# ETH3D/badslam

Measured on AMD Instinct MI355X. Metric: BA iterations/sec (and ms/iter) at N keyframes x M surfels, 640x480, higher is better.
Workload: dtype f32

## Files before the change

badslam_amd/capi.py:

```python
import ctypes as C
import os

_HERE = os.path.dirname(os.path.abspath(__file__))
LIB_PATH = os.path.join(os.environ.get("BADSLAM_LIB_DIR") or os.path.join(_HERE, "lib"), "libbadslam_hip.so")

SURFEL_ATTRIBUTE_COUNT = 17
MERGE_BUFFER_COUNT = 3
KF_ACTIVE, KF_COVISIBLE_ACTIVE, KF_INACTIVE = 0, 1, 2
ARITHMETIC_EXACT, ARITHMETIC_FAST = 0, 1

SURFEL_X, SURFEL_Y, SURFEL_Z, SURFEL_NORMAL, SURFEL_RADIUS_SQUARED, SURFEL_COLOR, SURFEL_DESCRIPTOR1, SURFEL_DESCRIPTOR2 = range(8)
SURFEL_ACCUM0 = 8


class BackendError(RuntimeError):
    pass


class Camera(C.Structure):
    _fields_ = [("fx", C.c_float), ("fy", C.c_float), ("cx", C.c_float), ("cy", C.c_float),
                ("width", C.c_int32), ("height", C.c_int32)]


class DepthParams(C.Structure):
# ... 186 lines not shown
                                             C.POINTER(C.c_uint32), C.POINTER(C.c_uint32)]),
    "bahip_extract_surfel_shard": (C.c_int, [C.c_void_p, C.POINTER(Surfels), C.c_int, C.c_int, C.c_uint32, C.POINTER(Surfels), C.POINTER(C.c_uint32)]),
    "bahip_debug_set_intrinsics_bin_capacity": (C.c_int, [C.c_void_p, C.c_int]),
    "bahip_debug_intrinsics_bin_stats": (C.c_int, [C.c_void_p, C.POINTER(C.c_uint32), C.POINTER(C.c_uint32), C.POINTER(C.c_uint64)]),
    "bahip_debug_set_intrinsics_slices": (C.c_int, [C.c_void_p, C.c_int]),
    "bahip_debug_read_intrinsics_sums": (C.c_int, [C.c_void_p, C.POINTER(C.c_float), C.POINTER(C.c_float)]),
    "bahip_exchange_stats": (C.c_int, [C.c_void_p, C.POINTER(C.c_longlong), C.POINTER(C.c_longlong), C.c_int]),
    "bahip_context_set_lifecycle_dealing": (C.c_int, [C.c_void_p, C.c_int]),
    "bahip_debug_lifecycle_deal_stats": (C.c_int, [C.c_void_p, C.POINTER(C.c_longlong), C.c_int]),
    "bahip_debug_exact_sum": (C.c_int, [C.c_void_p, C.POINTER(C.c_float), C.c_size_t, C.c_int, C.POINTER(C.c_double)]),
    "bahip_debug_count_pairs": (C.c_int, [C.c_void_p, C.POINTER(Surfels), C.POINTER(C.c_uint64)]),
    "bahip_debug_set_launch_shapes": (C.c_int, [C.c_int, C.c_int]),
    "bahip_debug_set_pose_form": (C.c_int, [C.c_int]),
    "bahip_debug_set_append_groups": (C.c_int, [C.c_int]),
    "bahip_debug_geometry_hybrid_launches": (C.c_int, [C.POINTER(C.c_longlong)]),
    "bahip_debug_set_creation_chain": (C.c_int, [C.c_int]),
    "bahip_debug_creation_chain_batches": (C.c_int, [C.POINTER(C.c_longlong)]),
    "bahip_debug_set_merge_cells": (C.c_int, [C.c_int]),
    "bahip_debug_merge_cells_batches": (C.c_int, [C.POINTER(C.c_longlong)]),
    "bahip_debug_set_pose_lds_items": (C.c_int, [C.c_int]),
    "bahip_debug_set_pose_lds_shape": (C.c_int, [C.c_int, C.c_int]),
    "bahip_debug_set_fused_iteration_begin": (C.c_int, [C.c_int]),
    "bahip_debug_set_intrinsics_reduce_form": (C.c_int, [C.c_int]),
    "bahip_debug_set_pose_rounds_ahead": (C.c_int, [C.c_int]),
    "bahip_debug_set_device_loop": (C.c_int, [C.c_int]),
    "bahip_debug_alternating_loop_calls": (C.c_int, [C.POINTER(C.c_longlong), C.POINTER(C.c_longlong)]),
    "bahip_debug_set_pcg_lds_form": (C.c_int, [C.c_int]),
    "bahip_debug_pose_form_launches": (C.c_int, [C.POINTER(C.c_longlong), C.POINTER(C.c_longlong), C.c_int]),
    "bahip_debug_pose_kernel_dispatches": (C.c_int, [C.POINTER(C.c_longlong)]),
    "bahip_debug_live_allocations": (C.c_int, [C.POINTER(C.c_longlong), C.POINTER(C.c_longlong)]),
# ... 40 lines not shown
```

badslam_amd/csrc/ba_launch.h:

```cpp
#pragma once

#include "ba_device.h"
#include <cstdlib>

inline int bahip_env_int(const char* name, int fallback) {
  const char* e = std::getenv(name);
  return e ? std::atoi(e) : fallback;
}

#ifdef BAHIP_FAST_MATH
#define BAHIP_FLAVOUR fast
#else
#define BAHIP_FLAVOUR exact
#endif
#define BAHIP_FLAVOURED_BEGIN namespace bahip { namespace BAHIP_FLAVOUR {
#define BAHIP_FLAVOURED_END } }

namespace bahip {

struct SupportingView {
  uint32_t* b[BAHIP_MERGE_BUFFER_COUNT];
  uint32_t pitch;
};

// ... 65 lines not shown
                       int update_activation, int round, void* host_out,
                       int sequence ,
                       const PoseLoopControl* loop = nullptr);
void launch_pose_init_from_keyframes(hipStream_t stream, const KfEntry* frames, int num_kfs, void* work, HbFixed* Hb, void* host_out,
                                     int kf_rank = 0, int kf_world = 1 ,
                                     const int* stop = nullptr);

void launch_window_activation(hipStream_t stream, KfEntry* frames, int num_kfs, const uint8_t* in_window, const int* offsets,
                              const int* indices, const int* stop = nullptr);
void launch_propagate_covisible(hipStream_t stream, KfEntry* frames, int num_kfs, const int* offsets, const int* indices,
                                const int* stop = nullptr);
bool launch_iteration_begin(hipStream_t stream, KfEntry* frames, int num_kfs, int mode, const uint8_t* in_window, const int* offsets, const int* indices,
                            void* work, HbFixed* Hb, void* host_out, const int* stop);

void set_tile_waves(int waves);
long long geometry_hybrid_launches();
void set_pose_lds_waves(int waves);
void set_pose_lds_parts_shift(int shift);
void set_pose_lds_items(int items);
void pcg_step1_form_launches(long long out[2]);
long long pose_kernel_dispatches();
void pose_form_launches(long long out[2], bool reset);
void set_pose_form(int form);
void set_pose_parts(int parts);
void launch_jacobian_debug(hipStream_t stream, int kind, const float* in, float* out);
void launch_pose_step_debug(hipStream_t stream, const float* in, float* out);
void launch_exact_math_debug(hipStream_t stream, int kind, const float* in, float* out, size_t n);
void launch_pose_limbs_debug(hipStream_t stream, const float* in, long long* out, size_t n);
void launch_wave_reduce_debug(hipStream_t stream, const float* in, float* out);
void launch_evaluate_pairs(hipStream_t stream, const Intrinsics& in, const KfEntry& frame, const SurfelsView& s,
// ... 170 lines not shown


#define BAHIP_FLAVOURED_DECLARATIONS                                                                                                          \
                                                                                                                      \
  void launch_activation(hipStream_t stream, const Intrinsics& in, const KfEntry* kfs, int num_kfs, const SurfelsView& s, uint32_t surfels_size); \
  void launch_normals(hipStream_t stream, const Intrinsics& in, const KfEntry* kfs, int num_kfs, const SurfelsView& s);                       \
  void launch_geometry(hipStream_t stream, bool use_depth, bool use_desc, const Intrinsics& in, const KfEntry* kfs, int num_kfs,              \
                       const SurfelsView& s, long long activate_count, const uint32_t* sched, const int* stop);                              \
  void launch_geometry_phase(hipStream_t stream, int phase, bool use_depth, bool use_desc, const Intrinsics& in, const KfEntry* kfs,          \
                             int num_kfs, const SurfelsView& s, long long activate_count, const ClassPartials& cpn, const ClassPartials& cpp); \
  void launch_activation_hits(hipStream_t stream, const Intrinsics& in, const KfEntry* kfs, int num_kfs, const SurfelsView& s,                \
                              uint32_t surfels_size, int kf_rank, int kf_world, uint32_t* hits);                                              \
  void launch_normals_phase(hipStream_t stream, int phase, const Intrinsics& in, const KfEntry* kfs, int num_kfs, const SurfelsView& s,      \
                            const ClassPartials& cp);                                                                                         \
  void set_tile_waves(int waves);                                                                                                             \
  long long geometry_hybrid_launches();                                                                                                       \
                                                                                                                        \
  void launch_pose_accumulate(hipStream_t stream, bool use_depth, bool use_desc, const Intrinsics& in, const KfEntry* frames,                 \
                              const void* work, int num_work, const SurfelsView& s, HbFixed* Hb, void* tile_bounds, bool stored_bounds,       \
                              int num_listed, uint32_t* tile_counters, int* parity_inout, uint32_t* tile_cost, const uint32_t* sched,         \
                              const int* listed_count, const int* stop);                                                                      \
  bool pose_round_can_be_queued_ahead(uint32_t surfels, int num_items, bool have_tile_counters);                                              \
  void set_pose_lds_waves(int waves);                                                                                                         \
  void set_pose_lds_parts_shift(int shift);                                                                                                   \
  void set_pose_lds_items(int items);                                                                                                         \
  long long pose_kernel_dispatches();                                                                                                         \
  void pose_form_launches(long long out[2], bool reset);                                                                                      \
  void set_pose_form(int form);                                                                                                               \
  void set_pose_parts(int parts);                                                                                                             \
  void launch_evaluate_pairs(hipStream_t stream, const Intrinsics& in, const KfEntry& frame, const SurfelsView& s, const uint32_t* indices,   \
// ... 77 lines not shown
```

badslam_amd/csrc/capi.hip:

```cpp
#include "capi_internal.h"

using namespace bahip;
using namespace bahip_capi;

namespace bahip_capi {

thread_local std::string g_last_error;

int fail(const char* what, const char* file, int line, hipError_t e) {
  char buf[512];
  if (e != hipSuccess) snprintf(buf, sizeof(buf), "%s failed at %s:%d: %s", what, file, line, hipGetErrorString(e));
  else snprintf(buf, sizeof(buf), "%s (%s:%d)", what, file, line);
  g_last_error = buf;
  return 1;
}

Intrinsics make_intrinsics(const bahip_camera& cc, const bahip_camera& dc, const bahip_depth_params& dp) {
  Intrinsics in{};
  in.fx = dc.fx; in.fy = dc.fy; in.cx = dc.cx; in.cy = dc.cy;
  in.fx_inv = 1.0f / dc.fx;
  in.fy_inv = 1.0f / dc.fy;
  const float cx_pixel_center = dc.cx - 0.5f, cy_pixel_center = dc.cy - 0.5f;
  in.cx_inv = -cx_pixel_center * in.fx_inv;
  in.cy_inv = -cy_pixel_center * in.fy_inv;
// ... 195 lines not shown
  if (!ctx) return;
  hipStreamSynchronize(ctx->stream);
#ifdef BAHIP_COUNT_CANDIDATES
  bahip::pose_counters_dump();
#endif
#ifdef BAHIP_TILE_TIMELINE
  if (const char* dir = getenv("BAHIP_TIMELINE_DIR")) {
    bahip::geometry_timeline_dump((std::string(dir) + "/geometry_timeline.bin").c_str());
    bahip::pose_timeline_dump((std::string(dir) + "/pose_timeline.bin").c_str());
  }
#endif
  if (ctx->intr_aux_stream) { hipStreamDestroy(ctx->intr_aux_stream); for (hipEvent_t e : ctx->intr_events) if (e) hipEventDestroy(e); }
  stage_free(&ctx->stage_kfs); stage_free(&ctx->stage_covis); stage_free(&ctx->stage_window); stage_free(&ctx->stage_gather);
  rccl_destroy_communicator(ctx);
  for (auto& t : ctx->timers) for (auto e : t.ev) hipEventDestroy(e);
  delete ctx;
}

int bahip_context_synchronize(bahip_context* ctx) {
  HIP_TRY(hipStreamSynchronize(ctx->stream));
  return 0;
}

int bahip_context_take_capacity_exceeded(bahip_context* ctx) {
  const int flag = ctx->capacity_exceeded ? 1 : 0;
  ctx->capacity_exceeded = false;
  return flag;
}

int bahip_malloc_pitch(void** ptr, size_t* pitch_bytes, size_t width_bytes, size_t height) {
// ... 292 lines not shown
```

badslam_amd/csrc/capi_debug.hip:

```cpp
#include "capi_internal.h"

using namespace bahip;
using namespace bahip_capi;

static const char* const kHookScratch = "the scratch of a test hook";

extern "C" {
int bahip_debug_live_allocations(long long* count_out, long long* bytes_out) {
  if (count_out) *count_out = g_live_allocations.load();
  if (bytes_out) *bytes_out = g_live_bytes.load();
  return 0;
}

int bahip_debug_evaluate_pairs(bahip_context* ctx, const bahip_frame* frame, const float frame_T_global[12],
                               const bahip_surfels* surfels, const uint32_t* surfel_indices_host, int count, float* out_host) {
  REQUIRE(ctx->have_intrinsics, "bahip_set_intrinsics not called");
  if (count <= 0) return 0;
  KfEntry e;
  if (make_entry(ctx, *frame, 0, &e)) return 1;
  memcpy(e.pose.F, frame_T_global, 12 * sizeof(float));
  DeviceBuffer<uint32_t> idx; DeviceBuffer<float> out;
  if (idx.reserve(count, 0, kHookScratch) || out.reserve(40 * (size_t)count, 0, kHookScratch)) return 1;
  HIP_TRY(hipMemcpy(idx, surfel_indices_host, sizeof(uint32_t) * count, hipMemcpyHostToDevice));
  launch_evaluate_pairs(ctx->stream, ctx->in, e, make_view(surfels), idx, count, out);
// ... 94 lines not shown
  REQUIRE(form == 0 || form == 1 || form == 2, "pose form must be 0 (automatic), 1 (one tile per wavefront, global atomics) or 2 (persistent, LDS table)");
  set_pose_form(form);
  return 0;
}

int bahip_debug_set_launch_shapes(int tile_waves, int pose_parts) {
  REQUIRE(tile_waves == 0 || tile_waves == 1 || tile_waves == 4 || tile_waves == 5, "tile_waves must be 0 (automatic), 1, 4 or 5 (the geometry step's hybrid shape)");
  REQUIRE(pose_parts == 0 || pose_parts == 1 || pose_parts == 2 || pose_parts == 4 || pose_parts == 8, "pose_parts must be 0, 1, 2, 4 or 8");
  set_tile_waves(tile_waves);
  set_pose_parts(pose_parts);
  return 0;
}

int bahip_debug_geometry_hybrid_launches(long long* launches_out) { if (launches_out) *launches_out = geometry_hybrid_launches(); return 0; }

int bahip_debug_jacobian(bahip_context* ctx, int kind, const float* in, int n_in, float* out, int n_out) {
  REQUIRE(kind >= 0 && kind <= 4 && n_in > 0 && n_in <= 16 && n_out > 0 && n_out <= 8, "bahip_debug_jacobian: bad arguments");
  DeviceBuffer<float> d_in, d_out;
  if (d_in.reserve(16, 0, kHookScratch) || d_out.reserve(8, 0, kHookScratch)) return 1;
  HIP_TRY(hipMemcpyAsync(d_in, in, n_in * sizeof(float), hipMemcpyHostToDevice, ctx->stream));
  launch_jacobian_debug(ctx->stream, kind, d_in, d_out);
  CHECK_LAUNCH();
  HIP_TRY(hipMemcpyAsync(out, d_out, n_out * sizeof(float), hipMemcpyDeviceToHost, ctx->stream));
  HIP_TRY(hipStreamSynchronize(ctx->stream));
  return 0;
}

int bahip_debug_read_pattern(bahip_context* ctx, size_t bytes, int pattern, int repeats) {
  REQUIRE(bytes >= 4096 && (pattern == 0 || pattern == 1) && repeats >= 1, "bahip_debug_read_pattern: bad arguments");
  DeviceBuffer<void> buf;
// ... 123 lines not shown
```

badslam_amd/csrc/capi_internal.h:

```cpp
#pragma once

#include <dlfcn.h>
#include <stdio.h>
#include <stdlib.h>
#include <string.h>

#include <atomic>
#include <chrono>
#include <memory>
#include <thread>

#include <string>
#include <vector>

#include "ba_launch.h"
#include "capi_buffers.h"
#include "exact_sum.h"
#include "ldlt.h"
#include "se3_device.h"

namespace bahip_capi {
using namespace bahip;

int fail(const char* what, const char* file, int line, hipError_t e = hipSuccess);
// ... 87 lines not shown
  DeviceBuffer<uint32_t> merge_planes[BAHIP_MERGE_BUFFER_COUNT];
  const void* supporting_planes_empty = nullptr;
  bool row_major_creation = false;
  bool poll_disabled = false;
  DeviceBuffer<void> dev_lifecycle_bounds;
  size_t lifecycle_bounds_capacity = 0;
  uint32_t lifecycle_bounds_tiles = 0;
  const void* lifecycle_bounds_data = nullptr;
  std::vector<float> lifecycle_frames;
  std::vector<uint32_t> lifecycle_list_offsets, lifecycle_list_counts;
  DeviceBuffer<float> dev_lifecycle_frames;
  DeviceBuffer<uint32_t> dev_lifecycle_cursors;
  DeviceBuffer<uint32_t> dev_lifecycle_lists;
  DeviceBuffer<void> dev_tile_bounds;
  DeviceBuffer<uint32_t> dev_tile_cost, dev_tile_order;
  size_t tile_schedule_capacity = 0;
  uint32_t tile_order_tiles = 0;
  int phases_since_schedule = 0;
  uint32_t tile_order_unavailable_tiles = 0;
  bool tile_order_unavailable_for(uint32_t padded_tiles) const { return padded_tiles != 0 && tile_order_unavailable_tiles == padded_tiles; }
  DeviceBuffer<int> dev_loop_ctl;
  PinnedBuffer<int> host_loop_ctl{kHostVisible};
  int rounds_hint_table = 1, rounds_hint_frame = 1;

  DeviceBuffer<void> intr_scratch;
  int intr_capacity = 0;
  DeviceBuffer<uint32_t> intr_bin_cursors;
  DeviceBuffer<uint32_t> intr_bin_records;
  PinnedBuffer<uint32_t> intr_bin_counts_host;
  int intr_bin_count = 0;
// ... 100 lines not shown
```

badslam_amd/csrc/kernels_surfel.hip:

```cpp
#include <stdlib.h>
#include <cstdio>

#include "ba_device.h"
#include "ba_launch.h"
#include "wave_cull.h"

namespace bahip {

#ifndef BAHIP_WAVES_ATTR
#define BAHIP_WAVES_ATTR __attribute__((amdgpu_waves_per_eu(4)))
#endif
constexpr int kSurfelBlock = 64;
constexpr int kMaxSumClasses = 8;

enum SumsMode { kSumsFused = 0, kSumsProduce = 1, kSumsConsume = 2 };
__device__ __forceinline__ bool position_valid(Vec3 p) { return p.x == p.x; }
static inline unsigned grid_for(uint32_t n) { return xcd_padded_tiles((n + kSurfelBlock - 1) / kSurfelBlock); }
#if defined(BAHIP_TILE_TIMELINE) && !defined(BAHIP_FAST_MATH)
__device__ unsigned long long g_geometry_timeline[65536][2];
void geometry_timeline_dump(const char* path) {
  static unsigned long long host[65536][2];
  if (hipMemcpyFromSymbol(host, HIP_SYMBOL(g_geometry_timeline), sizeof(host)) != hipSuccess) return;
  if (FILE* f = fopen(path, "wb")) { fwrite(host, sizeof(host), 1, f); fclose(f); }
}
// ... 75 lines not shown
  bool active = false;
  for_each_candidate_until(
      num_kfs,
      [&](int k) { return kfs[k].activation == BAHIP_KF_ACTIVE && sphere_may_project(in, kfs[k].pose.F, wb); },
      [&](int k) {
        if (in_range && !active) {
          Assoc r;
          if (project_associate<false>(in, kfs[k].pose.F, kfs[k].geom, gp, gn, &r, nullptr)) active = true;
        }
        return __all(active || !in_range) != 0;
      });
  if (in_range) s.active[i] = (s.active[i] & (uint8_t)~kSurfelActiveFlag) | (active ? kSurfelActiveFlag : 0);
}

constexpr int kMaskChunks = 4;
template <int kWaves, bool kActivate, int kMode = kSumsFused>
__device__ __forceinline__ void normals_pass(const Intrinsics& in, const KfEntry* __restrict__ kfs, int num_kfs,
                                             const WaveBounds& wb, SurfelsView& s, uint32_t i, bool* live_inout, bool decide,
                                             Vec3 gp, Vec3* gn_inout, float* lds, const ClassPartials& cp = ClassPartials{},
                                             bool in_range = false, unsigned long long* masks = nullptr) {
  const bool writer = kWaves == 1 || (threadIdx.x >> 6) == 0;
  const Vec3 gn = *gn_inout;
  bool live = *live_inout;
  constexpr int kCount = kActivate ? 5 : 4;
  float sum[kCount];
  tile_sums<kWaves, kCount, kMode>(sum, lds, [&](float (&acc)[kCount], int cls) {
    struct Started { Projected p; PixelWords pix; };
    for_each_candidate_pipelined<Started>(
        num_kfs,
        [&](int k) {
          float f[12];
          int32_t activation;
          load_candidate(kfs[k].pose.F, &kfs[k].activation, f, &activation);
          return activation != BAHIP_KF_INACTIVE && sphere_may_project(in, f, wb);
        },
        [&](int k) {
          Started st;
          st.p = project_surfel(in, kfs[k].pose.F, gp);
          st.pix = load_pixel_words(in, kfs[k].geom, st.p);
          return st;
        },
        [&](int k, const Started& st) {
          const Projected& p = st.p;
          const PixelWords& pix = st.pix;
          Assoc r;
          const bool associated = live && associate_from_words<false>(in, kfs[k].pose.F, gn, p, pix, &r, nullptr);
          gathers_arrived(pix);
          if (associated) {
            const Vec3 g = mul33(kfs[k].pose.GR, unpack_normal8(r.normal_bits));
            acc[0] += g.x; acc[1] += g.y; acc[2] += g.z; acc[3] += 1.f;
            if (kActivate) acc[kCount - 1] += (kfs[k].activation == BAHIP_KF_ACTIVE) ? 1.f : 0.f;
          }
        },
        in.sum_classes, cls, masks ? masks + cls * kMaskChunks : nullptr, masks ? kMaskChunks : 0, false);
  }, in.sum_classes, cp, i, in_range);
  if (kMode == kSumsProduce) return;
  if (kActivate && decide) {
    const bool active = live && sum[kCount - 1] >= 1.f;
    if (writer) s.active[i] = (s.active[i] & (uint8_t)~kSurfelActiveFlag) | (active ? kSurfelActiveFlag : 0);
    live = active;
    *live_inout = active;
  }
  if (!live) return;
  const float sx = sum[0], sy = sum[1], sz = sum[2], count = sum[3];
  if (count >= 1) {
    const uint32_t packed = pack_normal10((1.f / count) * mk3(sx, sy, sz));
    if (writer) reinterpret_cast<uint32_t*>(s.row(kSurfelNormal))[i] = packed;
    *gn_inout = unpack_normal10(packed);
  }
}

template <int kWaves>
__global__ void __launch_bounds__(64 * kWaves) BAHIP_WAVES_ATTR
normals_kernel(Intrinsics in, const KfEntry* __restrict__ kfs, int num_kfs, SurfelsView s) {
  __shared__ float lds[kWaves == 1 ? 1 : kMaxSumClasses * 4 * 64];
  const int lane = threadIdx.x & 63;
  const uint32_t i = xcd_chunked_tile(blockIdx.x) * kSurfelBlock + lane;
  const bool in_range = i < s.size;
  const uint32_t ii = in_range ? i : 0;
  bool live = in_range && (s.active[ii] & kSurfelActiveFlag);
  const Vec3 gp = surfel_position(s, ii);
  Vec3 gn = surfel_normal(s, ii);
  const WaveBounds wb = wave_bounds(gp, live && position_valid(gp));
  normals_pass<kWaves, false>(in, kfs, num_kfs, wb, s, ii, &live, false, gp, &gn, lds);
}

template <bool kUseDepth, bool kUseDesc, int kWaves, bool kActivate, int kPhase>
__device__ __forceinline__ void geometry_step(const Intrinsics& in, const KfEntry* __restrict__ kfs, int num_kfs, SurfelsView& s,
                                              uint32_t activate_count, float* lds, const ClassPartials& cpn, const ClassPartials& cpp,
                                              uint32_t tile , unsigned long long* replay_masks) {
  constexpr int kNormalsMode = kPhase == 1 ? kSumsProduce : kPhase == 2 ? kSumsConsume : kSumsFused;
  constexpr int kPositionMode = kPhase == 2 ? kSumsProduce : kPhase == 3 ? kSumsConsume : kSumsFused;
  const int lane = threadIdx.x & 63;
  const bool writer = kWaves == 1 || (threadIdx.x >> 6) == 0;
  const uint32_t i = tile * kSurfelBlock + lane;
  const bool in_range = i < s.size;
  const uint32_t ii = in_range ? i : 0;
  const bool decide = kActivate && kPhase != 3 && in_range && i < activate_count;
  bool live = in_range && (decide || (s.active[ii] & kSurfelActiveFlag));
  const Vec3 gp = surfel_position(s, ii);
  Vec3 gn = surfel_normal(s, ii);
  const WaveBounds wb = wave_bounds(gp, live && position_valid(gp));
  if (wb.r < 0.f) {
    if (decide && writer && kPhase != 1) s.active[ii] = s.active[ii] & (uint8_t)~kSurfelActiveFlag;
    return;
  }
  constexpr bool kReplayMasks = kWaves == 1 && kPhase == 0;
  unsigned long long* masks = kReplayMasks ? replay_masks : nullptr;
  if (kPhase != 3) normals_pass<kWaves, kActivate, kNormalsMode>(in, kfs, num_kfs, wb, s, ii, &live, decide, gp, &gn, lds, cpn, in_range, masks);
  if (kPhase == 1) return;

  auto cand = [&](int k) {
    float f[12];
    int32_t activation;
    load_candidate(kfs[k].pose.F, &kfs[k].activation, f, &activation);
    return activation != BAHIP_KF_INACTIVE && sphere_may_project(in, f, wb);
  };

  if (!kUseDesc) {
    float hb[2];
    tile_sums<kWaves, 2, kPositionMode>(hb, lds, [&](float (&acc)[2], int cls) {
      for_each_candidate_cached(num_kfs, cand, [&](int k) {
        const Projected p = project_surfel(in, kfs[k].pose.F, gp);
        const PixelWords pix = load_pixel_words(in, kfs[k].geom, p);
// ... 98 lines not shown
  const float x2 = y2 / H22;
  const float x1 = (y1 - H12 * x2) / H11;
  const float x0 = (y0 - H02 * x2 - H01 * x1) / H00;
  if (x0 != 0) {
    const Vec3 np = gp - x0 * gn;
    s.row(kSurfelX)[i] = np.x; s.row(kSurfelY)[i] = np.y; s.row(kSurfelZ)[i] = np.z;
  }
  if (x1 != 0) s.row(kSurfelDescriptor1)[i] = fmaxf(-180.f, fminf(180.f, d1 - x1));
  if (x2 != 0) s.row(kSurfelDescriptor2)[i] = fmaxf(-180.f, fminf(180.f, d2 - x2));
}


template <bool kUseDepth, bool kUseDesc, int kWaves, bool kActivate>
__global__ void __launch_bounds__(64 * kWaves) BAHIP_WAVES_ATTR
geometry_kernel(Intrinsics in, const KfEntry* __restrict__ kfs, int num_kfs, SurfelsView s, uint32_t activate_count,
                const uint32_t* __restrict__ sched, const int* __restrict__ stop ) {
  __shared__ float lds[kWaves == 1 ? 1 : kMaxSumClasses * 8 * 64];
  __shared__ unsigned long long candidate_masks[kWaves == 1 ? kMaxSumClasses * kMaskChunks : 1];
  if (stop && load_global(stop) != 0) return;
#ifdef BAHIP_RECORD_GEOMETRY_TIMELINE
  const unsigned long long t0 = wall_clock64();
#endif
  uint32_t tile;
  if (!scheduled_tile(blockIdx.x, gridDim.x - (sched ? kHeavySlots : 0u), sched, &tile)) return;
  geometry_step<kUseDepth, kUseDesc, kWaves, kActivate, 0>(in, kfs, num_kfs, s, activate_count, lds, ClassPartials{}, ClassPartials{}, tile, candidate_masks);
#ifdef BAHIP_RECORD_GEOMETRY_TIMELINE
  if (threadIdx.x == 0 && blockIdx.x < 65536) { g_geometry_timeline[blockIdx.x][0] = t0; g_geometry_timeline[blockIdx.x][1] = wall_clock64(); }
#endif
}

#ifndef BAHIP_HYBRID_WAVES
#define BAHIP_HYBRID_WAVES 4
#endif
template <bool kUseDepth, bool kUseDesc, bool kActivate>
__global__ void __launch_bounds__(256) __attribute__((amdgpu_waves_per_eu(BAHIP_HYBRID_WAVES)))
geometry_hybrid_kernel(Intrinsics in, const KfEntry* __restrict__ kfs, int num_kfs, SurfelsView s, uint32_t activate_count,
                       const uint32_t* __restrict__ sched , uint32_t padded_tiles, const int* __restrict__ stop) {
  __shared__ float lds[kMaxSumClasses * 8 * 64];
  __shared__ unsigned long long candidate_masks[4][kMaxSumClasses * kMaskChunks];
  if (stop && load_global(stop) != 0) return;
// ... 51 lines not shown
          if (project_associate<false>(in, kfs[k].pose.F, kfs[k].geom, gp, gn, &r, nullptr)) active = true;
        }
        return __all(active || !in_range) != 0;
      });
  if (in_range) hits[i] = active ? 1u : 0u;
}
void launch_activation(hipStream_t stream, const Intrinsics& in, const KfEntry* kfs, int num_kfs, const SurfelsView& s,
                       uint32_t surfels_size) {
  if (surfels_size == 0) return;
  hipLaunchKernelGGL(activation_kernel, dim3(grid_for(surfels_size)), dim3(kSurfelBlock), 0, stream, in, kfs, num_kfs, s,
                     surfels_size);
}

static int g_forced_tile_waves = bahip_env_int("BAHIP_TILE_WAVES", 0);
static long long g_geometry_hybrid_launches = 0;
long long geometry_hybrid_launches() { return g_geometry_hybrid_launches; }
void set_tile_waves(int waves) { g_forced_tile_waves = waves; }
static int tile_waves(uint32_t surfels) {
  const int forced = g_forced_tile_waves;
  if (forced == 1 || forced == 4) return forced;
  return grid_for(surfels) >= 8192 ? 1 : 4;
}

void launch_normals(hipStream_t stream, const Intrinsics& in, const KfEntry* kfs, int num_kfs, const SurfelsView& s) {
  if (s.size == 0) return;
  const dim3 grid(grid_for(s.size));
  switch (tile_waves(s.size)) {
    case 1: hipLaunchKernelGGL(normals_kernel<1>, grid, dim3(64), 0, stream, in, kfs, num_kfs, s); break;
    default: hipLaunchKernelGGL(normals_kernel<4>, grid, dim3(256), 0, stream, in, kfs, num_kfs, s); break;
  }
}

template <int kWaves, bool kActivate>
static void launch_geometry_shape(hipStream_t stream, bool use_depth, bool use_desc, const Intrinsics& in, const KfEntry* kfs,
                                  int num_kfs, const SurfelsView& s, uint32_t activate_count, const uint32_t* sched, const int* stop) {
  const dim3 grid(sched_positions(grid_for(s.size), sched)), block(64 * kWaves);
  if (!use_desc) hipLaunchKernelGGL((geometry_kernel<true, false, kWaves, kActivate>), grid, block, 0, stream, in, kfs, num_kfs, s, activate_count, sched, stop);
  else if (use_depth) hipLaunchKernelGGL((geometry_kernel<true, true, kWaves, kActivate>), grid, block, 0, stream, in, kfs, num_kfs, s, activate_count, sched, stop);
  else hipLaunchKernelGGL((geometry_kernel<false, true, kWaves, kActivate>), grid, block, 0, stream, in, kfs, num_kfs, s, activate_count, sched, stop);
}

template <bool kActivate>
static void launch_geometry_hybrid(hipStream_t stream, bool use_depth, bool use_desc, const Intrinsics& in, const KfEntry* kfs,
                                   int num_kfs, const SurfelsView& s, uint32_t activate_count, const uint32_t* sched, const int* stop) {
  const uint32_t padded = grid_for(s.size);
  const dim3 grid(kHeavySlots + (padded + 3u) / 4u), block(256);
  if (!use_desc) hipLaunchKernelGGL((geometry_hybrid_kernel<true, false, kActivate>), grid, block, 0, stream, in, kfs, num_kfs, s, activate_count, sched, padded, stop);
  else if (use_depth) hipLaunchKernelGGL((geometry_hybrid_kernel<true, true, kActivate>), grid, block, 0, stream, in, kfs, num_kfs, s, activate_count, sched, padded, stop);
  else hipLaunchKernelGGL((geometry_hybrid_kernel<false, true, kActivate>), grid, block, 0, stream, in, kfs, num_kfs, s, activate_count, sched, padded, stop);
}

void launch_geometry(hipStream_t stream, bool use_depth, bool use_desc, const Intrinsics& in, const KfEntry* kfs,
                     int num_kfs, const SurfelsView& s, long long activate_count, const uint32_t* sched, const int* stop) {
  if (s.size == 0) return;
// ... 141 lines not shown
                     long long activate_count, const uint32_t* sched, const int* stop) {
  BAHIP_PICK(in, launch_geometry(stream, use_depth, use_desc, in, kfs, num_kfs, s, activate_count, sched, stop));
}
void launch_geometry_phase(hipStream_t stream, int phase, bool use_depth, bool use_desc, const Intrinsics& in, const KfEntry* kfs, int num_kfs,
                           const SurfelsView& s, long long activate_count, const ClassPartials& cpn, const ClassPartials& cpp) {
  BAHIP_PICK(in, launch_geometry_phase(stream, phase, use_depth, use_desc, in, kfs, num_kfs, s, activate_count, cpn, cpp));
}
void launch_normals_phase(hipStream_t stream, int phase, const Intrinsics& in, const KfEntry* kfs, int num_kfs, const SurfelsView& s, const ClassPartials& cp) {
  BAHIP_PICK(in, launch_normals_phase(stream, phase, in, kfs, num_kfs, s, cp));
}
void launch_activation_hits(hipStream_t stream, const Intrinsics& in, const KfEntry* kfs, int num_kfs, const SurfelsView& s, uint32_t surfels_size,
                            int kf_rank, int kf_world, uint32_t* hits) {
  BAHIP_PICK(in, launch_activation_hits(stream, in, kfs, num_kfs, s, surfels_size, kf_rank, kf_world, hits));
}
void set_tile_waves(int waves) { exact::set_tile_waves(waves); fast::set_tile_waves(waves); }
long long geometry_hybrid_launches() { return exact::geometry_hybrid_launches() + fast::geometry_hybrid_launches(); }
}

namespace bahip {
__global__ void __launch_bounds__(kSurfelBlock) BAHIP_WAVES_ATTR
count_pairs_kernel(Intrinsics in, const KfEntry* __restrict__ kfs, int num_kfs, SurfelsView s, unsigned long long* counts) {
  const uint32_t i = xcd_chunked_tile(blockIdx.x) * kSurfelBlock + threadIdx.x;
  const bool in_range = i < s.size;
  const uint32_t ii = in_range ? i : 0;
  const Vec3 gp = surfel_position(s, ii);
  const Vec3 gn = surfel_normal(s, ii);
  const WaveBounds wb = wave_bounds(gp, in_range && position_valid(gp));
  unsigned long long cand = 0, wave_hits = 0, lane_hits = 0, in_image = 0;
  for_each_candidate(
      num_kfs, [&](int k) { return sphere_may_project_item(in, kfs[k].pose.F, wb); },
// ... 20 lines not shown
```

badslam_amd/csrc/wave_cull.h:

```cpp
#pragma once

#include "ba_device.h"

namespace bahip {

constexpr uint32_t kXcdLargeGrid = 32768;
__host__ __device__ __forceinline__ uint32_t xcd_padded_tiles(uint32_t tiles) {
  uint32_t padded = (tiles + 255u) / 256u * 256u;
  if (padded >= kXcdLargeGrid) padded = (tiles + 1023u) / 1024u * 1024u;
  return padded;
}
__device__ __forceinline__ uint32_t xcd_chunked_tile(uint32_t block) {
  const uint32_t shift = gridDim.x >= kXcdLargeGrid ? 7u : 5u;
  const uint32_t xcd = block & 7u, j = block >> 3;
  return ((((j >> shift) << 3) + xcd) << shift) + (j & ((1u << shift) - 1u));
}

__device__ __forceinline__ uint32_t xcd_chunked_tile_of(uint32_t block, uint32_t padded_tiles) {
  const uint32_t shift = padded_tiles >= kXcdLargeGrid ? 7u : 5u;
  const uint32_t xcd = block & 7u, j = block >> 3;
  return ((((j >> shift) << 3) + xcd) << shift) + (j & ((1u << shift) - 1u));
}

constexpr uint32_t kHeavySlots = 1024;
// ... 143 lines not shown
    if (!m) continue;
    int k = base + __builtin_ctzll(m) * parts;
    m &= m - 1;
    State state = issue(k);
    while (m) {
      const int next = base + __builtin_ctzll(m) * parts;
      m &= m - 1;
      State ahead = issue(next);
      consume(k, state);
      k = next;
      state = ahead;
    }
    consume(k, state);
  }
}
template <typename Pred, typename Body>
__device__ __forceinline__ void for_each_candidate_until(int num_items, Pred pred, Body body) {
  const int lane = threadIdx.x & 63;
  for (int base = 0; base < num_items; base += 64) {
    const int item = base + lane;
    const bool cand = (item < num_items) && pred(item);
    unsigned long long m = __ballot(cand);
    while (m) {
      const int k = base + __builtin_ctzll(m);
      m &= m - 1;
      if (body(k)) return;
    }
  }
}

// ... 2 lines not shown
```

include/badslam_hip.h:

```cpp
#ifndef BADSLAM_HIP_H_
#define BADSLAM_HIP_H_

#include <stddef.h>
#include <stdint.h>

#ifdef __cplusplus
extern "C" {
#endif

#define BAHIP_SURFEL_ATTRIBUTE_COUNT 17
#define BAHIP_MERGE_BUFFER_COUNT 3
#define BAHIP_MAX_POSE_ITERATIONS 30

enum { BAHIP_KF_ACTIVE = 0, BAHIP_KF_COVISIBLE_ACTIVE = 1, BAHIP_KF_INACTIVE = 2 };

typedef struct bahip_camera {
  float fx, fy, cx, cy;
  int32_t width, height;
} bahip_camera;

typedef struct bahip_depth_params {
  float a;
  float raw_to_float_depth;
  float baseline_fx;
// ... 243 lines not shown
                                             const bahip_pose_step_control* control, const bahip_surfels* surfels, int update_activation,
                                             float* lambda_inout, float* global_T_frame_out, int* iterations_done, int* converged, int* moved,
                                             int* trials_out, int* rejected_out, bahip_cost* cost_before_out, bahip_cost* cost_after_out,
                                             int* rounds_out, int* num_converged_out);
int bahip_debug_pose_step_damped(bahip_context* ctx, const float* H21_b6, const float* global_T_frame, float lambda, float* out_25);

int bahip_debug_evaluate_pairs(bahip_context* ctx, const bahip_frame* frame, const float frame_T_global[12],
                               const bahip_surfels* surfels, const uint32_t* surfel_indices, int count, float* out);

int bahip_debug_read_pcg_vector(bahip_context* ctx, int which, size_t offset, size_t count, float* out);

int bahip_debug_exact_sum(bahip_context* ctx, const float* values, size_t count, int mode, double* out);

int bahip_debug_set_launch_shapes(int tile_waves, int pose_parts);
int bahip_debug_geometry_hybrid_launches(long long* launches_out);
int bahip_debug_set_pose_form(int form);
int bahip_debug_set_tile_order(int enabled);
int bahip_debug_read_tile_schedule(bahip_context* ctx, uint32_t* padded_tiles_out, uint32_t* words_out, size_t max_words);
int bahip_debug_set_intrinsics_bin_capacity(bahip_context* ctx, int records_per_block);
int bahip_debug_intrinsics_bin_stats(bahip_context* ctx, uint32_t* capacity_out, uint32_t* most_out, uint64_t* total_out);
int bahip_debug_read_intrinsics_sums(bahip_context* ctx, float out[34], float* cells_out);
int bahip_debug_set_intrinsics_slices(bahip_context* ctx, int slices);
int bahip_debug_set_append_groups(int groups);
int bahip_debug_set_creation_chain(int enabled);
int bahip_debug_creation_chain_batches(long long* batches_out);
int bahip_debug_set_merge_cells(int enabled);
int bahip_debug_merge_cells_batches(long long* batches_out);
int bahip_debug_set_pose_lds_items(int items);
int bahip_debug_set_pose_lds_shape(int waves, int parts_shift);
int bahip_debug_set_pose_rounds_ahead(int rounds);
// ... 32 lines not shown
```

Measured before the change: 748.0.

## Prune replayed keyframe candidate masks for the position pass using normal-pass association results

```diff
diff --git a/badslam_amd/capi.py b/badslam_amd/capi.py
--- a/badslam_amd/capi.py
+++ b/badslam_amd/capi.py
@@ -224,6 +224,8 @@
     "bahip_debug_set_pose_form": (C.c_int, [C.c_int]),
     "bahip_debug_set_append_groups": (C.c_int, [C.c_int]),
     "bahip_debug_geometry_hybrid_launches": (C.c_int, [C.POINTER(C.c_longlong)]),
+    "bahip_debug_set_geometry_pruning": (C.c_int, [C.c_int]),
+    "bahip_debug_geometry_prune_counts": (C.c_int, [C.c_void_p, C.c_int, C.POINTER(C.c_uint64)]),
     "bahip_debug_set_creation_chain": (C.c_int, [C.c_int]),
     "bahip_debug_creation_chain_batches": (C.c_int, [C.POINTER(C.c_longlong)]),
     "bahip_debug_set_merge_cells": (C.c_int, [C.c_int]),
diff --git a/badslam_amd/csrc/ba_launch.h b/badslam_amd/csrc/ba_launch.h
--- a/badslam_amd/csrc/ba_launch.h
+++ b/badslam_amd/csrc/ba_launch.h
@@ -103,6 +103,9 @@
                             void* work, HbFixed* Hb, void* host_out, const int* stop);
 
 void set_tile_waves(int waves);
+void set_geometry_pruning(int enabled);
+void set_geometry_prune_stats(unsigned long long* stats);
+const unsigned long long* geometry_prune_stats();
 long long geometry_hybrid_launches();
 void set_pose_lds_waves(int waves);
 void set_pose_lds_parts_shift(int shift);
@@ -303,6 +306,8 @@
   void launch_normals_phase(hipStream_t stream, int phase, const Intrinsics& in, const KfEntry* kfs, int num_kfs, const SurfelsView& s,      \
                             const ClassPartials& cp);                                                                                         \
   void set_tile_waves(int waves);                                                                                                             \
+  void set_geometry_pruning(int enabled);                                                                                                     \
+  void set_geometry_prune_stats(unsigned long long* stats);                                                                                   \
   long long geometry_hybrid_launches();                                                                                                       \
                                                                                                                         \
   void launch_pose_accumulate(hipStream_t stream, bool use_depth, bool use_desc, const Intrinsics& in, const KfEntry* frames,                 \
diff --git a/badslam_amd/csrc/capi.hip b/badslam_amd/csrc/capi.hip
--- a/badslam_amd/csrc/capi.hip
+++ b/badslam_amd/csrc/capi.hip
@@ -233,6 +233,7 @@
   stage_free(&ctx->stage_kfs); stage_free(&ctx->stage_covis); stage_free(&ctx->stage_window); stage_free(&ctx->stage_gather);
   rccl_destroy_communicator(ctx);
   for (auto& t : ctx->timers) for (auto e : t.ev) hipEventDestroy(e);
+  if (ctx->geometry_prune_stats && bahip::geometry_prune_stats() == ctx->geometry_prune_stats.get()) bahip::set_geometry_prune_stats(nullptr);
   delete ctx;
 }
 
diff --git a/badslam_amd/csrc/capi_debug.hip b/badslam_amd/csrc/capi_debug.hip
--- a/badslam_amd/csrc/capi_debug.hip
+++ b/badslam_amd/csrc/capi_debug.hip
@@ -132,6 +132,29 @@
 
 int bahip_debug_geometry_hybrid_launches(long long* launches_out) { if (launches_out) *launches_out = geometry_hybrid_launches(); return 0; }
 
+int bahip_debug_set_geometry_pruning(int enabled) { set_geometry_pruning(enabled); return 0; }
+
+int bahip_debug_geometry_prune_counts(bahip_context* ctx, int collect, uint64_t* counts_out) {
+  const bool collecting = ctx->geometry_prune_stats && geometry_prune_stats() == ctx->geometry_prune_stats.get();
+  if (counts_out) {
+    memset(counts_out, 0, 4 * sizeof(uint64_t));
+    if (collecting) {
+      HIP_TRY(hipDeviceSynchronize());
+      HIP_TRY(hipMemcpy(counts_out, ctx->geometry_prune_stats, 4 * sizeof(unsigned long long), hipMemcpyDeviceToHost));
+    }
+  }
+  if (collect) {
+    if (ctx->geometry_prune_stats.reserve(4, 0, "the counters of the pruned position pass")) return 1;
+    HIP_TRY(hipMemset(ctx->geometry_prune_stats, 0, 4 * sizeof(unsigned long long)));
+    set_geometry_prune_stats(ctx->geometry_prune_stats);
+  } else if (collecting) {
+    HIP_TRY(hipDeviceSynchronize());
+    set_geometry_prune_stats(nullptr);
+    ctx->geometry_prune_stats.release();
+  }
+  return 0;
+}
+
 int bahip_debug_jacobian(bahip_context* ctx, int kind, const float* in, int n_in, float* out, int n_out) {
   REQUIRE(kind >= 0 && kind <= 4 && n_in > 0 && n_in <= 16 && n_out > 0 && n_out <= 8, "bahip_debug_jacobian: bad arguments");
   DeviceBuffer<float> d_in, d_out;
diff --git a/badslam_amd/csrc/capi_internal.h b/badslam_amd/csrc/capi_internal.h
--- a/badslam_amd/csrc/capi_internal.h
+++ b/badslam_amd/csrc/capi_internal.h
@@ -125,6 +125,7 @@
   DeviceBuffer<uint32_t> dev_lifecycle_lists;
   DeviceBuffer<void> dev_tile_bounds;
   DeviceBuffer<uint32_t> dev_tile_cost, dev_tile_order;
+  DeviceBuffer<unsigned long long> geometry_prune_stats;
   size_t tile_schedule_capacity = 0;
   uint32_t tile_order_tiles = 0;
   int phases_since_schedule = 0;
diff --git a/badslam_amd/csrc/kernels_surfel.hip b/badslam_amd/csrc/kernels_surfel.hip
--- a/badslam_amd/csrc/kernels_surfel.hip
+++ b/badslam_amd/csrc/kernels_surfel.hip
@@ -113,45 +113,59 @@
 }
 
 constexpr int kMaskChunks = 4;
-template <int kWaves, bool kActivate, int kMode = kSumsFused>
+constexpr int kMaskWords = kMaxSumClasses * kMaskChunks;
+template <int kWaves, bool kActivate, int kMode = kSumsFused, bool kPrune = false>
 __device__ __forceinline__ void normals_pass(const Intrinsics& in, const KfEntry* __restrict__ kfs, int num_kfs,
                                              const WaveBounds& wb, SurfelsView& s, uint32_t i, bool* live_inout, bool decide,
                                              Vec3 gp, Vec3* gn_inout, float* lds, const ClassPartials& cp = ClassPartials{},
-                                             bool in_range = false, unsigned long long* masks = nullptr) {
+                                             bool in_range = false, unsigned long long* masks = nullptr, bool* changed_out = nullptr) {
+  static_assert(!kPrune || (kWaves == 1 && kMode == kSumsFused), "pruned masks: the one-wavefront whole-step form only");
   const bool writer = kWaves == 1 || (threadIdx.x >> 6) == 0;
   const Vec3 gn = *gn_inout;
   bool live = *live_inout;
+  if (kPrune) *changed_out = false;
   constexpr int kCount = kActivate ? 5 : 4;
   float sum[kCount];
   tile_sums<kWaves, kCount, kMode>(sum, lds, [&](float (&acc)[kCount], int cls) {
     struct Started { Projected p; PixelWords pix; };
-    for_each_candidate_pipelined<Started>(
-        num_kfs,
-        [&](int k) {
-          float f[12];
-          int32_t activation;
-          load_candidate(kfs[k].pose.F, &kfs[k].activation, f, &activation);
-          return activation != BAHIP_KF_INACTIVE && sphere_may_project(in, f, wb);
-        },
-        [&](int k) {
-          Started st;
-          st.p = project_surfel(in, kfs[k].pose.F, gp);
-          st.pix = load_pixel_words(in, kfs[k].geom, st.p);
-          return st;
-        },
-        [&](int k, const Started& st) {
-          const Projected& p = st.p;
-          const PixelWords& pix = st.pix;
-          Assoc r;
-          const bool associated = live && associate_from_words<false>(in, kfs[k].pose.F, gn, p, pix, &r, nullptr);
-          gathers_arrived(pix);
-          if (associated) {
-            const Vec3 g = mul33(kfs[k].pose.GR, unpack_normal8(r.normal_bits));
-            acc[0] += g.x; acc[1] += g.y; acc[2] += g.z; acc[3] += 1.f;
-            if (kActivate) acc[kCount - 1] += (kfs[k].activation == BAHIP_KF_ACTIVE) ? 1.f : 0.f;
-          }
-        },
-        in.sum_classes, cls, masks ? masks + cls * kMaskChunks : nullptr, masks ? kMaskChunks : 0, false);
+    auto pred = [&](int k) {
+      float f[12];
+      int32_t activation;
+      load_candidate(kfs[k].pose.F, &kfs[k].activation, f, &activation);
+      return activation != BAHIP_KF_INACTIVE && sphere_may_project(in, f, wb);
+    };
+    auto issue = [&](int k) {
+      Started st;
+      st.p = project_surfel(in, kfs[k].pose.F, gp);
+      st.pix = load_pixel_words(in, kfs[k].geom, st.p);
+      return st;
+    };
+    auto consume = [&](int k, const Started& st) {
+      const Projected& p = st.p;
+      const PixelWords& pix = st.pix;
+      Assoc r;
+      const bool associated = live && associate_from_words<false>(in, kfs[k].pose.F, gn, p, pix, &r, nullptr);
+      gathers_arrived(pix);
+      if (associated) {
+        const Vec3 g = mul33(kfs[k].pose.GR, unpack_normal8(r.normal_bits));
+        acc[0] += g.x; acc[1] += g.y; acc[2] += g.z; acc[3] += 1.f;
+        if (kActivate) acc[kCount - 1] += (kfs[k].activation == BAHIP_KF_ACTIVE) ? 1.f : 0.f;
+      }
+      return associated;
+    };
+    if constexpr (kPrune) {
+      for_each_candidate_pipelined_pruning<Started>(
+          num_kfs, pred, issue,
+          [&](int k, const Started& st) {
+            const bool associated = consume(k, st);
+            const bool before_normal = live && st.p.ok && !((uint16_t)(st.pix.geom & 0xffffu) & kInvalidDepthBit);
+            return (__ballot(associated) != 0 ? 1u : 0u) | (__ballot(before_normal) != 0 ? 2u : 0u);
+          },
+          in.sum_classes, cls, masks + cls * kMaskChunks, kMaskChunks, kMaskWords);
+    } else {
+      for_each_candidate_pipelined<Started>(num_kfs, pred, issue, [&](int k, const Started& st) { consume(k, st); }, in.sum_classes, cls,
+                                            masks ? masks + cls * kMaskChunks : nullptr, masks ? kMaskChunks : 0, false);
+    }
   }, in.sum_classes, cp, i, in_range);
   if (kMode == kSumsProduce) return;
   if (kActivate && decide) {
@@ -165,7 +179,10 @@
   if (count >= 1) {
     const uint32_t packed = pack_normal10((1.f / count) * mk3(sx, sy, sz));
     if (writer) reinterpret_cast<uint32_t*>(s.row(kSurfelNormal))[i] = packed;
-    *gn_inout = unpack_normal10(packed);
+    const Vec3 updated = unpack_normal10(packed);
+    *gn_inout = updated;
+    if (kPrune) *changed_out = __float_as_uint(updated.x) != __float_as_uint(gn.x) || __float_as_uint(updated.y) != __float_as_uint(gn.y) ||
+                               __float_as_uint(updated.z) != __float_as_uint(gn.z);
   }
 }
 
@@ -184,10 +201,11 @@
   normals_pass<kWaves, false>(in, kfs, num_kfs, wb, s, ii, &live, false, gp, &gn, lds);
 }
 
-template <bool kUseDepth, bool kUseDesc, int kWaves, bool kActivate, int kPhase>
+template <bool kUseDepth, bool kUseDesc, int kWaves, bool kActivate, int kPhase, bool kPrune = false>
 __device__ __forceinline__ void geometry_step(const Intrinsics& in, const KfEntry* __restrict__ kfs, int num_kfs, SurfelsView& s,
                                               uint32_t activate_count, float* lds, const ClassPartials& cpn, const ClassPartials& cpp,
-                                              uint32_t tile , unsigned long long* replay_masks) {
+                                              uint32_t tile , unsigned long long* replay_masks,
+                                              int prune = 0, unsigned long long* prune_stats = nullptr) {
   constexpr int kNormalsMode = kPhase == 1 ? kSumsProduce : kPhase == 2 ? kSumsConsume : kSumsFused;
   constexpr int kPositionMode = kPhase == 2 ? kSumsProduce : kPhase == 3 ? kSumsConsume : kSumsFused;
   const int lane = threadIdx.x & 63;
@@ -206,7 +224,26 @@
   }
   constexpr bool kReplayMasks = kWaves == 1 && kPhase == 0;
   unsigned long long* masks = kReplayMasks ? replay_masks : nullptr;
-  if (kPhase != 3) normals_pass<kWaves, kActivate, kNormalsMode>(in, kfs, num_kfs, wb, s, ii, &live, decide, gp, &gn, lds, cpn, in_range, masks);
+  static_assert(!kPrune || kReplayMasks, "pruned masks are replayed masks");
+  if constexpr (kPrune) {
+    bool changed;
+    normals_pass<kWaves, kActivate, kNormalsMode, true>(in, kfs, num_kfs, wb, s, ii, &live, decide, gp, &gn, lds, cpn, in_range, masks, &changed);
+    const bool unchanged = __ballot(changed) == 0;
+    const int copy = prune ? (unchanged ? 1 : 2) : 0;
+    if (prune_stats != nullptr && lane == 0) {
+      unsigned long long full = 0, kept = 0;
+      for (int c = 0; c < in.sum_classes; ++c)
+        for (int chunk = 0; chunk < kMaskChunks && c + chunk * 64 * in.sum_classes < num_kfs; ++chunk) {
+          full += __popcll(masks[c * kMaskChunks + chunk]);
+          kept += __popcll(masks[copy * kMaskWords + c * kMaskChunks + chunk]);
+        }
+      atomicAdd(&prune_stats[0], 1ull); atomicAdd(&prune_stats[1], unchanged ? 1ull : 0ull);
+      atomicAdd(&prune_stats[2], full); atomicAdd(&prune_stats[3], full - kept);
+    }
+    masks += copy * kMaskWords;
+  } else if (kPhase != 3) {
+    normals_pass<kWaves, kActivate, kNormalsMode>(in, kfs, num_kfs, wb, s, ii, &live, decide, gp, &gn, lds, cpn, in_range, masks);
+  }
   if (kPhase == 1) return;
 
   auto cand = [&](int k) {
@@ -335,16 +372,18 @@
 template <bool kUseDepth, bool kUseDesc, int kWaves, bool kActivate>
 __global__ void __launch_bounds__(64 * kWaves) BAHIP_WAVES_ATTR
 geometry_kernel(Intrinsics in, const KfEntry* __restrict__ kfs, int num_kfs, SurfelsView s, uint32_t activate_count,
-                const uint32_t* __restrict__ sched, const int* __restrict__ stop ) {
+                const uint32_t* __restrict__ sched, const int* __restrict__ stop ,
+                int prune, unsigned long long* prune_stats ) {
   __shared__ float lds[kWaves == 1 ? 1 : kMaxSumClasses * 8 * 64];
-  __shared__ unsigned long long candidate_masks[kWaves == 1 ? kMaxSumClasses * kMaskChunks : 1];
+  __shared__ unsigned long long candidate_masks[kWaves == 1 ? 3 * kMaskWords : 1];
   if (stop && load_global(stop) != 0) return;
 #ifdef BAHIP_RECORD_GEOMETRY_TIMELINE
   const unsigned long long t0 = wall_clock64();
 #endif
   uint32_t tile;
   if (!scheduled_tile(blockIdx.x, gridDim.x - (sched ? kHeavySlots : 0u), sched, &tile)) return;
-  geometry_step<kUseDepth, kUseDesc, kWaves, kActivate, 0>(in, kfs, num_kfs, s, activate_count, lds, ClassPartials{}, ClassPartials{}, tile, candidate_masks);
+  geometry_step<kUseDepth, kUseDesc, kWaves, kActivate, 0, kWaves == 1>(in, kfs, num_kfs, s, activate_count, lds, ClassPartials{}, ClassPartials{}, tile,
+                                                                        candidate_masks, prune, prune_stats);
 #ifdef BAHIP_RECORD_GEOMETRY_TIMELINE
   if (threadIdx.x == 0 && blockIdx.x < 65536) { g_geometry_timeline[blockIdx.x][0] = t0; g_geometry_timeline[blockIdx.x][1] = wall_clock64(); }
 #endif
@@ -426,6 +465,10 @@
 
 static int g_forced_tile_waves = bahip_env_int("BAHIP_TILE_WAVES", 0);
 static long long g_geometry_hybrid_launches = 0;
+static int g_geometry_prune = bahip_env_int("BAHIP_GEOMETRY_PRUNE", 1) != 0 ? 1 : 0;
+static unsigned long long* g_geometry_prune_stats = nullptr;
+void set_geometry_pruning(int enabled) { g_geometry_prune = enabled ? 1 : 0; }
+void set_geometry_prune_stats(unsigned long long* stats) { g_geometry_prune_stats = stats; }
 long long geometry_hybrid_launches() { return g_geometry_hybrid_launches; }
 void set_tile_waves(int waves) { g_forced_tile_waves = waves; }
 static int tile_waves(uint32_t surfels) {
@@ -447,9 +490,9 @@
 static void launch_geometry_shape(hipStream_t stream, bool use_depth, bool use_desc, const Intrinsics& in, const KfEntry* kfs,
                                   int num_kfs, const SurfelsView& s, uint32_t activate_count, const uint32_t* sched, const int* stop) {
   const dim3 grid(sched_positions(grid_for(s.size), sched)), block(64 * kWaves);
-  if (!use_desc) hipLaunchKernelGGL((geometry_kernel<true, false, kWaves, kActivate>), grid, block, 0, stream, in, kfs, num_kfs, s, activate_count, sched, stop);
-  else if (use_depth) hipLaunchKernelGGL((geometry_kernel<true, true, kWaves, kActivate>), grid, block, 0, stream, in, kfs, num_kfs, s, activate_count, sched, stop);
-  else hipLaunchKernelGGL((geometry_kernel<false, true, kWaves, kActivate>), grid, block, 0, stream, in, kfs, num_kfs, s, activate_count, sched, stop);
+  if (!use_desc) hipLaunchKernelGGL((geometry_kernel<true, false, kWaves, kActivate>), grid, block, 0, stream, in, kfs, num_kfs, s, activate_count, sched, stop, g_geometry_prune, g_geometry_prune_stats);
+  else if (use_depth) hipLaunchKernelGGL((geometry_kernel<true, true, kWaves, kActivate>), grid, block, 0, stream, in, kfs, num_kfs, s, activate_count, sched, stop, g_geometry_prune, g_geometry_prune_stats);
+  else hipLaunchKernelGGL((geometry_kernel<false, true, kWaves, kActivate>), grid, block, 0, stream, in, kfs, num_kfs, s, activate_count, sched, stop, g_geometry_prune, g_geometry_prune_stats);
 }
 
 template <bool kActivate>
@@ -621,6 +664,13 @@
   BAHIP_PICK(in, launch_activation_hits(stream, in, kfs, num_kfs, s, surfels_size, kf_rank, kf_world, hits));
 }
 void set_tile_waves(int waves) { exact::set_tile_waves(waves); fast::set_tile_waves(waves); }
+static unsigned long long* g_registered_prune_stats = nullptr;
+void set_geometry_pruning(int enabled) { exact::set_geometry_pruning(enabled); fast::set_geometry_pruning(enabled); }
+void set_geometry_prune_stats(unsigned long long* stats) {
+  g_registered_prune_stats = stats;
+  exact::set_geometry_prune_stats(stats); fast::set_geometry_prune_stats(stats);
+}
+const unsigned long long* geometry_prune_stats() { return g_registered_prune_stats; }
 long long geometry_hybrid_launches() { return exact::geometry_hybrid_launches() + fast::geometry_hybrid_launches(); }
 }
 
diff --git a/badslam_amd/csrc/wave_cull.h b/badslam_amd/csrc/wave_cull.h
--- a/badslam_amd/csrc/wave_cull.h
+++ b/badslam_amd/csrc/wave_cull.h
@@ -181,6 +181,45 @@
     consume(k, state);
   }
 }
+template <typename State, typename Pred, typename Issue, typename Consume>
+__device__ __forceinline__ void for_each_candidate_pipelined_pruning(int num_items, Pred pred, Issue issue, Consume consume, int parts, int part,
+                                                                     unsigned long long* masks, int max_masks, int pruned_stride) {
+  const int lane = threadIdx.x & 63;
+  int chunk = 0;
+  for (int base = part; base < num_items; base += 64 * parts, ++chunk) {
+    const int item = base + lane * parts;
+    const bool cand = (item < num_items) && pred(item);
+    const unsigned long long all = __ballot(cand);
+    unsigned long long keep0 = 0, keep1 = 0;
+    if (all) {
+      unsigned long long m = all;
+      unsigned long long bit = m & (0ull - m);
+      int k = base + __builtin_ctzll(m) * parts;
+      m &= m - 1;
+      State state = issue(k);
+      while (m) {
+        const unsigned long long next_bit = m & (0ull - m);
+        const int next = base + __builtin_ctzll(m) * parts;
+        m &= m - 1;
+        State ahead = issue(next);
+        const unsigned keep = consume(k, state);
+        keep0 |= (keep & 1u) ? bit : 0ull;
+        keep1 |= (keep & 2u) ? bit : 0ull;
+        k = next;
+        bit = next_bit;
+        state = ahead;
+      }
+      const unsigned keep = consume(k, state);
+      keep0 |= (keep & 1u) ? bit : 0ull;
+      keep1 |= (keep & 2u) ? bit : 0ull;
+    }
+    if (chunk < max_masks && lane == 0) {
+      masks[chunk] = all;
+      masks[pruned_stride + chunk] = keep0;
+      masks[2 * pruned_stride + chunk] = keep1;
+    }
+  }
+}
 template <typename Pred, typename Body>
 __device__ __forceinline__ void for_each_candidate_until(int num_items, Pred pred, Body body) {
   const int lane = threadIdx.x & 63;
diff --git a/include/badslam_hip.h b/include/badslam_hip.h
--- a/include/badslam_hip.h
+++ b/include/badslam_hip.h
@@ -281,6 +281,8 @@
 
 int bahip_debug_set_launch_shapes(int tile_waves, int pose_parts);
 int bahip_debug_geometry_hybrid_launches(long long* launches_out);
+int bahip_debug_set_geometry_pruning(int enabled);
+int bahip_debug_geometry_prune_counts(bahip_context* ctx, int collect, uint64_t* counts_out);
 int bahip_debug_set_pose_form(int form);
 int bahip_debug_set_tile_order(int enabled);
 int bahip_debug_read_tile_schedule(bahip_context* ctx, uint32_t* padded_tiles_out, uint32_t* words_out, size_t max_words);
```

Result: no change. 741.2 (-0.9%).
